# RViMLab/MICCAI2021_Cataract_semantic_segmentation

Hardware: AMD Instinct MI355X
Metric: train frames/sec @540x960 OCRNet-HRNetw48 (higher is better)
Workload: dtype f32 (convolutions with K >= 2048 and >= 192 output columns, and the 3x3 trunk convolutions of the HRNet widths: forward / backward-data of those with > 192 output columns: operands scaled by a per-tensor power of two and split into 2 fp16 planes (22 significant bits), 3 fp16 MFMA products; forward /

## Files before the change

miccai2021_cataract_semantic_segmentation_amd/csrc/pconv1.hip:

```cpp
#include "common.h"

namespace {

typedef _Float16 half8 __attribute__((ext_vector_type(8)));
typedef unsigned short u16;

__host__ __device__ inline int p1_exponent(unsigned amax_bits) {
  const int ex = (int)((amax_bits >> 23) & 0xFF);
  if (ex == 0 || ex == 255) return 0;
  const int e = 14 - (ex - 127);
  return e < -100 ? -100 : (e > 100 ? 100 : e);
}

__host__ __device__ constexpr int p1_bn(int N) { return N >= 256 ? 256 : (N + 31) / 32 * 32; }
__host__ __device__ constexpr int p1_ntn(int N) { return (N + p1_bn(N) - 1) / p1_bn(N); }
__host__ __device__ constexpr int p1_groups(int K) { return ((K + 31) / 32 + 1) / 2 * 2; }

struct P1Entry { long long w_off, img_off; int O, I, kh, kw, transposed, ky0, kys, nky, kx0, kxs, nkx, pad; };

__global__ __launch_bounds__(256) void p1_amax_batch_kernel(const float* __restrict__ flat, const P1Entry* __restrict__ ent, unsigned* __restrict__ recs) {
  const P1Entry e = ent[blockIdx.y];
  const float* w = flat + e.w_off;
  const long long n = (long long)e.O * e.I * e.kh * e.kw;
  unsigned m = 0;
  for (long long i = blockIdx.x * (long long)blockDim.x + threadIdx.x; i < n; i += (long long)gridDim.x * blockDim.x)
    m = max(m, __float_as_uint(w[i]) & 0x7FFFFFFFu);
  cs_amax_commit1(m, recs + 2 * blockIdx.y);
}

__global__ __launch_bounds__(256) void p1_prep_batch_kernel(const float* __restrict__ flat, const P1Entry* __restrict__ ent,
                                                            unsigned char* __restrict__ img_base, unsigned* __restrict__ recs) {
  const P1Entry e = ent[blockIdx.y];
  const int ex = p1_exponent(recs[2 * blockIdx.y]);
  if (blockIdx.x == 0 && threadIdx.x == 0) ((int*)recs)[2 * blockIdx.y + 1] = ex;
  const float* w = flat + e.w_off;
  const int N = e.transposed ? e.I : e.O, Ck = e.transposed ? e.O : e.I, K = e.nky * e.nkx * Ck;
  const int BN = p1_bn(N), ntn = p1_ntn(N), G = p1_groups(K);
  half8* img = (half8*)(img_base + e.img_off);
  const long long pieces = (long long)G * ntn * 2 * BN * 2;
  for (long long i = blockIdx.x * (long long)blockDim.x + threadIdx.x; i < pieces; i += (long long)gridDim.x * blockDim.x) {
    const int c = (int)(i & 1);
    long long r = i >> 1;
    const int nn = (int)(r % BN); r /= BN;
    const int kt = (int)(r & 1); r >>= 1;
    const int nt = (int)(r % ntn);
    const int g = (int)(r / ntn);
    const int n = nt * BN + nn, k0 = 32 * g + 16 * kt + 8 * c;
    half8 h, l;
#pragma unroll
    for (int j = 0; j < 8; ++j) {
      const int k = k0 + j;
      float v = 0.f;
      if (n < N && k < K) {
        const int t = k / Ck, c = k - t * Ck;
        const int ta = t / e.nkx, tb = t - ta * e.nkx;
        const int ky = e.ky0 + ta * e.kys, kx = e.kx0 + tb * e.kxs;
        const int o = e.transposed ? c : n, ci = e.transposed ? n : c;
        v = w[(((long long)o * e.kh + ky) * e.kw + kx) * e.I + ci];
      }
      const float xs = __builtin_ldexpf(v, ex);
      const _Float16 hh = (_Float16)xs;
      h[j] = hh;
      l[j] = (_Float16)(xs - (float)hh);
    }
    const int pc = c ^ ((nn >> 3) & 1);
    const long long row0 = (((long long)(g * ntn + nt) * 2 + kt) * 2) * BN;
    img[(row0 + nn) * 2 + pc] = h;
    img[(row0 + BN + nn) * 2 + pc] = l;
  }
}

struct P1Geo {
  int Wg, HWg;
  int si, y0, x0;
  int ya, xa, nb;
  int Hi, Wi, C;
  unsigned mC, mnb;
  int so, oy, ox, Ho, Wo;
  int linear_out;
};

struct P1Args {
  const float* x; int ldx;
  const unsigned* xrec;
  const unsigned char* wimg;
  const int* wrec;
  float* y; int ldy;
  const float* bias;
  int M, N, K;
  int tilesM, ntn;
  int accumulate;
  float* bn_part;
  unsigned long long x_bytes, img_bytes;
  unsigned long long y_bytes;
  P1Geo geo;
};

template <int NS>
__device__ __forceinline__ void p1_full_tile_bn_partials(float* lds, int tile_cols, int l31, bool writer_lane, int wave_m, const f32x16 (&acc)[NS],
                                                         float* part, int C, int gcol0) {
  constexpr int WM = 8;
  float mean[NS];
#pragma unroll
  for (int j = 0; j < NS; ++j) {
    float a = 0.f;
#pragma unroll
    for (int i = 0; i < 16; ++i) a += acc[j][i];
    a += __shfl_xor(a, 32, 64);
    if (writer_lane) lds[wave_m * tile_cols + 32 * j + l31] = a;
    __builtin_amdgcn_sched_barrier(0);
  }
  __syncthreads();
  const float inv = 1.f / 256.f;
#pragma unroll
  for (int j = 0; j < NS; ++j) {
    float t = 0.f;
#pragma unroll
    for (int w = 0; w < WM; ++w) t += lds[w * tile_cols + 32 * j + l31];
    mean[j] = t * inv;
  }
  __syncthreads();
#pragma unroll
  for (int j = 0; j < NS; ++j) {
    float a = 0.f, b = 0.f;
#pragma unroll
    for (int i = 0; i < 16; ++i) {
      const float d = acc[j][i] - mean[j];
      a += d;
      b += d * d;
    }
    a += __shfl_xor(a, 32, 64);
    b += __shfl_xor(b, 32, 64);
    if (writer_lane) {
      lds[wave_m * tile_cols + 32 * j + l31] = a;
      lds[(WM + wave_m) * tile_cols + 32 * j + l31] = b;
    }
    __builtin_amdgcn_sched_barrier(0);
  }
  __syncthreads();
  if (writer_lane && wave_m == 0) {
#pragma unroll
    for (int j = 0; j < NS; ++j) {
      const int gc = gcol0 + 32 * j + l31;
      if (gc < C) {
        float a = 0.f, b = 0.f;
#pragma unroll
        for (int w = 0; w < WM; ++w) {
          a += lds[w * tile_cols + 32 * j + l31];
          b += lds[(WM + w) * tile_cols + 32 * j + l31];
        }
        part[gc] = mean[j];
        part[C + gc] = a;
        part[2 * C + gc] = b;
      }
    }
  }
}

constexpr int p1_waitcnt(int vm) { return (vm & 15) | (7 << 4) | (15 << 8) | ((vm >> 4) << 14); }

template <int NT, bool GEO, bool FULL>
__device__ __forceinline__ void p1_body(const P1Args& p) {
  constexpr int BN = 32 * NT;
  constexpr int GB = 4 * BN * 32;
  constexpr int PIECES = GB / 16;
  constexpr int PB = (PIECES + 511) / 512;
  constexpr int NBUF = 3;
  constexpr int EPI = 2 * 8 * BN * 4;
  constexpr int SMEM = (NBUF * GB > EPI ? NBUF * GB : EPI) + 1024;
  __shared__ __attribute__((aligned(16))) char smem[SMEM];

  const int tid = threadIdx.x;
  const int lane = tid & 63;
  const int wave = __builtin_amdgcn_readfirstlane(tid >> 6);
  const int l31 = lane & 31, hh = lane >> 5;

  int tile_m = blockIdx.x, tile_n = 0;
  if (p.ntn > 1) {
    const int per = 8 * p.ntn, grp = blockIdx.x / per, r = blockIdx.x - grp * per;
    tile_n = r >> 3;
    tile_m = grp * 8 + (r & 7);
  }
  if (tile_m >= p.tilesM) return;
  const int m0 = tile_m * 256, n0 = tile_n * BN;

  const int ex = p1_exponent(cs_amax_read(p.xrec));
  const int G = p1_groups(p.K);

  f32x16 acc[NT];
#pragma unroll
  for (int u = 0; u < NT; ++u)
#pragma unroll
    for (int r = 0; r < 16; ++r) acc[u][r] = 0.f;

  const __amdgpu_buffer_rsrc_t rsA = __builtin_amdgcn_make_buffer_rsrc((void*)p.x, (short)0, (int)(unsigned)p.x_bytes, 0x00020000);
  const __amdgpu_buffer_rsrc_t rsB = __builtin_amdgcn_make_buffer_rsrc((void*)p.wimg, (short)0, (int)(unsigned)p.img_bytes, 0x00020000);
  constexpr unsigned OOB = 0xFFFFFFF0u;
  const int row = m0 + wave * 32 + l31;
  const unsigned klim = row < p.M ? (unsigned)p.K : 0u;
  unsigned a_row = 0;
  int ybase = 0, xbase = 0;
  if (GEO) {
    const int rr = row < p.M ? row : 0;
    const int gb = rr / p.geo.HWg, rem = rr - gb * p.geo.HWg;
    const int gi = rem / p.geo.Wg, gj = rem - gi * p.geo.Wg;
    ybase = gi * p.geo.si + p.geo.y0;
    xbase = gj * p.geo.si + p.geo.x0;
    a_row = (unsigned)(gb * p.geo.Hi * p.geo.Wi);
  } else {
    a_row = (unsigned)row * (unsigned)p.ldx * 4u + (unsigned)hh * 32u;
  }
  auto a_off = [&](int g, int kt, int c) -> unsigned {
    const unsigned k8 = (unsigned)(32 * g + 16 * kt + 8 * hh);
    if (GEO) {
      const unsigned tap = __umulhi(k8, p.geo.mC), cc = k8 - tap * (unsigned)p.geo.C;
      const unsigned ta = p.geo.nb == 1 ? tap : __umulhi(tap, p.geo.mnb), tb = tap - ta * (unsigned)p.geo.nb;
      const int yi = ybase + (int)ta * p.geo.ya, xi = xbase + (int)tb * p.geo.xa;
      const bool ok = (int)(k8 + 4u * c < klim) & (int)((unsigned)yi < (unsigned)p.geo.Hi) & (int)((unsigned)xi < (unsigned)p.geo.Wi);
      const unsigned m = (unsigned)-(int)ok;
      const unsigned off = ((a_row + (unsigned)(yi * p.geo.Wi + xi)) * (unsigned)p.ldx + cc) * 4u + 16u * c;
      return (off & m) | (OOB & ~m);
    }
    const unsigned m = (unsigned)-(int)(k8 + 4u * c < klim);
    return ((a_row + (unsigned)(32 * g + 16 * kt) * 4u + 16u * c) & m) | (OOB & ~m);
  };
  const unsigned b_lane = (unsigned)(wave * 64 + lane) * 16u;
  auto issueB = [&](int g, int buf) {
    const unsigned src0 = (unsigned)((g * p.ntn + tile_n)) * (unsigned)GB;
#pragma unroll
    for (int i = 0; i < PB; ++i) {
      const bool live = i * 512 + wave * 64 < PIECES;
      const unsigned voff = live ? src0 + (unsigned)i * 8192u + b_lane : OOB;
      char* dst = live ? smem + buf * GB + (i * 512 + wave * 64) * 16 : smem + SMEM - 1024;
      __builtin_amdgcn_raw_ptr_buffer_load_lds(rsB, (__attribute__((address_space(3))) void*)dst, 16, voff, 0, 0, 0);
    }
  };

  f32x4 ra[2][4];
  auto loadA = [&](int g, int par) {
#pragma unroll
    for (int q = 0; q < 4; ++q) ra[par][q] = __builtin_bit_cast(f32x4, __builtin_amdgcn_raw_buffer_load_b128(rsA, a_off(g, q >> 1, q & 1), 0, 0));
  };
  half8 Ah[2], Al[2];
  auto splitA = [&](int par) {
#pragma unroll
    for (int kt = 0; kt < 2; ++kt) {
      const f32x4 v0 = ra[par][kt * 2], v1 = ra[par][kt * 2 + 1];
#pragma unroll
      for (int j = 0; j < 8; ++j) {
        const float xs = __builtin_ldexpf(j < 4 ? v0[j & 3] : v1[j & 3], ex);
        const _Float16 h = (_Float16)xs;
        Ah[kt][j] = h;
        Al[kt][j] = (_Float16)(xs - (float)h);
      }
    }
  };
  const int boff = l31 * 32 + ((hh ^ ((l31 >> 3) & 1)) << 4);
  constexpr int NP = (NT + 1) / 2;
  auto compute = [&](int buf) {
    const char* bb = smem + buf * GB + boff;
    half8 bh[2][2], bl[2][2];
    auto rd = [&](int q, int st) {
      const int kt = q / NP, u = 2 * (q - kt * NP);
      bh[st][0] = *(const half8*)(bb + ((kt * 2 + 0) * BN + 32 * u) * 32);
      bl[st][0] = *(const half8*)(bb + ((kt * 2 + 1) * BN + 32 * u) * 32);
      if (u + 1 < NT) {
        bh[st][1] = *(const half8*)(bb + ((kt * 2 + 0) * BN + 32 * (u + 1)) * 32);
        bl[st][1] = *(const half8*)(bb + ((kt * 2 + 1) * BN + 32 * (u + 1)) * 32);
      }
    };
    rd(0, 0);
#pragma unroll
    for (int q = 0; q < 2 * NP; ++q) {
      const int st = q & 1, kt = q / NP, u = 2 * (q - kt * NP);
      if (q + 1 < 2 * NP) rd(q + 1, st ^ 1);
      if (u + 1 < NT) {
        acc[u] = __builtin_amdgcn_mfma_f32_32x32x16_f16(Al[kt], bh[st][0], acc[u], 0, 0, 0);
        acc[u + 1] = __builtin_amdgcn_mfma_f32_32x32x16_f16(Al[kt], bh[st][1], acc[u + 1], 0, 0, 0);
        acc[u] = __builtin_amdgcn_mfma_f32_32x32x16_f16(Ah[kt], bh[st][0], acc[u], 0, 0, 0);
        acc[u + 1] = __builtin_amdgcn_mfma_f32_32x32x16_f16(Ah[kt], bh[st][1], acc[u + 1], 0, 0, 0);
        acc[u] = __builtin_amdgcn_mfma_f32_32x32x16_f16(Ah[kt], bl[st][0], acc[u], 0, 0, 0);
        acc[u + 1] = __builtin_amdgcn_mfma_f32_32x32x16_f16(Ah[kt], bl[st][1], acc[u + 1], 0, 0, 0);
      } else {
        acc[u] = __builtin_amdgcn_mfma_f32_32x32x16_f16(Al[kt], bh[st][0], acc[u], 0, 0, 0);
        acc[u] = __builtin_amdgcn_mfma_f32_32x32x16_f16(Ah[kt], bh[st][0], acc[u], 0, 0, 0);
        acc[u] = __builtin_amdgcn_mfma_f32_32x32x16_f16(Ah[kt], bl[st][0], acc[u], 0, 0, 0);
      }
      __builtin_amdgcn_sched_barrier(0);
    }
  };

  loadA(0, 0);
  issueB(0, 0);
  loadA(1, 1);
  issueB(1, 1);
  for (int g = 0; g < G; g += 2) {
#pragma unroll
    for (int par = 0; par < 2; ++par) {
      const int gg = g + par;
      splitA(par);
      loadA(gg + 2, par);
      __builtin_amdgcn_sched_barrier(0);
      __builtin_amdgcn_s_waitcnt(p1_waitcnt(8 + PB));
      __builtin_amdgcn_s_barrier();
      asm volatile("" ::: "memory");
      issueB(gg + 2, (gg + 2) % NBUF);
      compute(gg % NBUF);
    }
  }
  __builtin_amdgcn_s_waitcnt(p1_waitcnt(0));
  __syncthreads();

  if constexpr (FULL) {
    const int ew_u = __builtin_amdgcn_readfirstlane(p.wrec[1]), ex_u = __builtin_amdgcn_readfirstlane(ex);
    const int es = -(ex_u + ew_u);
    if (es >= -120 && es <= 120) {
#pragma unroll
      for (int u = 0; u < NT; ++u)
#pragma unroll
        for (int r = 0; r < 16; ++r) acc[u][r] = __builtin_ldexpf(acc[u][r], es);
    } else {
#pragma unroll
      for (int u = 0; u < NT; ++u)
#pragma unroll
        for (int r = 0; r < 16; ++r) acc[u][r] = __builtin_ldexpf(__builtin_ldexpf(acc[u][r], -ex_u), -ew_u);
    }
    if (p.bias != nullptr) {
#pragma unroll
      for (int u = 0; u < NT; ++u) {
        const int col = n0 + 32 * u + l31;
        const float b = col < p.N ? p.bias[col] : 0.f;
#pragma unroll
        for (int r = 0; r < 16; ++r) acc[u][r] += b;
      }
    }
    if (p.bn_part != nullptr)
      p1_full_tile_bn_partials<NT>((float*)smem, BN, l31, hh == 0, wave, acc, p.bn_part + (long long)tile_m * 3 * p.N, p.N, n0);
    constexpr unsigned OOBS = 0xFFFFFFF0u;
    const bool accum = p.accumulate != 0;
    if (GEO && !p.geo.linear_out) {
      const __amdgpu_buffer_rsrc_t rsY = __builtin_amdgcn_make_buffer_rsrc((void*)p.y, (short)0, (int)(unsigned)p.y_bytes, 0x00020000);
      unsigned cb[NT];
#pragma unroll
      for (int u = 0; u < NT; ++u) cb[u] = n0 + 32 * u + l31 < p.N ? (unsigned)(n0 + 32 * u + l31) * 4u : OOBS;
#pragma unroll
      for (int r = 0; r < 16; ++r) {
        const int rw = m0 + wave * 32 + 4 * hh + (r & 3) + 8 * (r >> 2);
        const int gb = rw / p.geo.HWg, rem = rw - gb * p.geo.HWg;
        const int gi = rem / p.geo.Wg, gj = rem - gi * p.geo.Wg;
        const unsigned ro = rw < p.M ? (unsigned)((gb * p.geo.Ho + gi * p.geo.so + p.geo.oy) * p.geo.Wo + gj * p.geo.so + p.geo.ox) * (unsigned)p.ldy * 4u : OOBS;
        float v[NT];
#pragma unroll
        for (int u = 0; u < NT; ++u) v[u] = acc[u][r];
        if (accum) {
          float o[NT];
#pragma unroll
          for (int u = 0; u < NT; ++u) o[u] = __uint_as_float(__builtin_amdgcn_raw_buffer_load_b32(rsY, (cb[u] == OOBS || ro == OOBS) ? OOBS : ro + cb[u], 0, 0));
#pragma unroll
          for (int u = 0; u < NT; ++u) v[u] += o[u];
        }
#pragma unroll
        for (int u = 0; u < NT; ++u) __builtin_amdgcn_raw_buffer_store_b32(__float_as_uint(v[u]), rsY, (cb[u] == OOBS || ro == OOBS) ? OOBS : ro + cb[u], 0, 0);
        __builtin_amdgcn_sched_barrier(0);
      }
      return;
    }
    const unsigned rows_here = (unsigned)(p.M - m0 < 256 ? p.M - m0 : 256);
    const __amdgpu_buffer_rsrc_t rsY = __builtin_amdgcn_make_buffer_rsrc((void*)(p.y + (long long)m0 * p.ldy + n0), (short)0,
                                                                        (int)(rows_here * (unsigned)p.ldy * 4u - (unsigned)n0 * 4u), 0x00020000);
    const int ld4 = p.ldy * 4;
    const int voff = (wave * 32 + 4 * hh) * ld4 + l31 * 4;
    int vo[NT];
#pragma unroll
    for (int u = 0; u < NT; ++u) vo[u] = n0 + 32 * u + l31 < p.N ? voff + 128 * u : (int)OOBS;
#pragma unroll
    for (int r = 0; r < 16; ++r) {
      const int soff = ((r & 3) + 8 * (r >> 2)) * ld4;
      float v[NT];
#pragma unroll
      for (int u = 0; u < NT; ++u) v[u] = acc[u][r];
      if (accum) {
        float o[NT];
#pragma unroll
        for (int u = 0; u < NT; ++u) o[u] = __uint_as_float(__builtin_amdgcn_raw_buffer_load_b32(rsY, vo[u], soff, 0));
#pragma unroll
        for (int u = 0; u < NT; ++u) v[u] += o[u];
      }
#pragma unroll
      for (int u = 0; u < NT; ++u) __builtin_amdgcn_raw_buffer_store_b32(__float_as_uint(v[u]), rsY, vo[u], soff, 0);
      __builtin_amdgcn_sched_barrier(0);
    }
    return;
  }

  {
    const int ea = -ex, ew = -p.wrec[1];
#pragma unroll
    for (int u = 0; u < NT; ++u)
#pragma unroll
      for (int r = 0; r < 16; ++r) acc[u][r] = __builtin_ldexpf(__builtin_ldexpf(acc[u][r], ea), ew);
  }
  float bv[NT];
#pragma unroll
  for (int u = 0; u < NT; ++u) {
    const int col = n0 + 32 * u + l31;
    bv[u] = (p.bias != nullptr && col < p.N) ? p.bias[col] : 0.f;
  }
  const int rbase = m0 + wave * 32 + 4 * hh;
  if (p.bn_part != nullptr) {
    int colv[NT];
#pragma unroll
    for (int u = 0; u < NT; ++u) colv[u] = 32 * u + l31;
    cs_tile_bn_partials<NT, 16, 8, false>(
        (float*)smem, BN, colv, hh == 0, wave, min(256, p.M - m0),
        [&](int j, int i) { return acc[j][i] + bv[j]; },
        [&](int i) { return rbase + (i & 3) + 8 * (i >> 2) < p.M; }, p.bn_part + (long long)tile_m * 3 * p.N, p.N, n0);
  }
  long long orow[16];
#pragma unroll
  for (int r = 0; r < 16; ++r) {
    const int rw = rbase + (r & 3) + 8 * (r >> 2);
    if (GEO && !p.geo.linear_out) {
      const int rr = rw < p.M ? rw : 0;
      const int gb = rr / p.geo.HWg, rem = rr - gb * p.geo.HWg;
      const int gi = rem / p.geo.Wg, gj = rem - gi * p.geo.Wg;
      orow[r] = ((long long)(gb * p.geo.Ho + gi * p.geo.so + p.geo.oy) * p.geo.Wo + gj * p.geo.so + p.geo.ox) * p.ldy;
    } else {
      orow[r] = (long long)rw * p.ldy;
    }
  }
#pragma unroll
  for (int u = 0; u < NT; ++u) {
    const int col = n0 + 32 * u + l31;
    float add[16];
#pragma unroll
    for (int r = 0; r < 16; ++r) {
      const int rw = rbase + (r & 3) + 8 * (r >> 2);
      add[r] = (p.accumulate && rw < p.M && col < p.N) ? p.y[orow[r] + col] : 0.f;
    }
#pragma unroll
    for (int r = 0; r < 16; ++r) {
      const int rw = rbase + (r & 3) + 8 * (r >> 2);
      if (rw < p.M && col < p.N) p.y[orow[r] + col] = (acc[u][r] + bv[u]) + add[r];
    }
  }
}

template <int NT, bool GEO, bool FULL>
__global__ __launch_bounds__(512) void p1_kernel(const P1Args p) {
  p1_body<NT, GEO, FULL>(p);
}
struct P1Multi { P1Args a[4]; };
template <int NT, bool FULL>
__global__ __launch_bounds__(512) void p1_multi_kernel(const P1Multi q) {
  p1_body<NT, true, FULL>(q.a[blockIdx.y]);
}

template <int NT>
void p1_launch_multi(const P1Multi& q, int n, hipStream_t st) {
  int blocks = 0;
  bool full = true;
  for (int i = 0; i < n; ++i) {
    const P1Args& a = q.a[i];
    const int b = a.ntn > 1 ? (a.tilesM + 7) / 8 * 8 * a.ntn : a.tilesM;
    blocks = b > blocks ? b : blocks;
    const bool gathered = !a.geo.linear_out;
    full = full && (gathered ? (a.y_bytes > 0 && a.y_bytes < 0xFFFFFFF0ull) : (a.M % 256 == 0 || a.bn_part == nullptr));
  }
  if (full) hipLaunchKernelGGL((p1_multi_kernel<NT, true>), dim3(blocks, n), dim3(512), 0, st, q);
  else hipLaunchKernelGGL((p1_multi_kernel<NT, false>), dim3(blocks, n), dim3(512), 0, st, q);
}
void p1_dispatch_multi(const P1Multi& q, int n, hipStream_t st) {
  switch (p1_bn(q.a[0].N) / 32) {
    case 1: p1_launch_multi<1>(q, n, st); break;
    case 2: p1_launch_multi<2>(q, n, st); break;
    case 3: p1_launch_multi<3>(q, n, st); break;
    case 4: p1_launch_multi<4>(q, n, st); break;
    case 5: p1_launch_multi<5>(q, n, st); break;
    case 6: p1_launch_multi<6>(q, n, st); break;
    case 7: p1_launch_multi<7>(q, n, st); break;
    default: p1_launch_multi<8>(q, n, st); break;
  }
}

template <int NT>
void p1_launch(const P1Args& a, bool geo, hipStream_t st) {
  const int per = 8 * a.ntn;
  const int blocks = a.ntn > 1 ? (a.tilesM + 7) / 8 * per : a.tilesM;
  const bool gathered = geo && !a.geo.linear_out;
  const bool full = gathered ? (a.y_bytes > 0 && a.y_bytes < 0xFFFFFFF0ull) : (a.M % 256 == 0 || a.bn_part == nullptr);
  if (geo) {
    if (full) hipLaunchKernelGGL((p1_kernel<NT, true, true>), dim3(blocks), dim3(512), 0, st, a);
    else hipLaunchKernelGGL((p1_kernel<NT, true, false>), dim3(blocks), dim3(512), 0, st, a);
  } else {
    if (full) hipLaunchKernelGGL((p1_kernel<NT, false, true>), dim3(blocks), dim3(512), 0, st, a);
    else hipLaunchKernelGGL((p1_kernel<NT, false, false>), dim3(blocks), dim3(512), 0, st, a);
  }
}

void p1_dispatch(const P1Args& a, bool geo, hipStream_t st) {
  switch (p1_bn(a.N) / 32) {
    case 1: p1_launch<1>(a, geo, st); break;
    case 2: p1_launch<2>(a, geo, st); break;
    case 3: p1_launch<3>(a, geo, st); break;
    case 4: p1_launch<4>(a, geo, st); break;
    case 5: p1_launch<5>(a, geo, st); break;
    case 6: p1_launch<6>(a, geo, st); break;
    case 7: p1_launch<7>(a, geo, st); break;
    default: p1_launch<8>(a, geo, st); break;
  }
}

struct P1TArgs {
  const float* dy; int lddy; const unsigned* dyrec;
  const float* x; int ldx; const unsigned* xrec;
  float* slabs;
  long long P;
  int M, N;
  int nbn, Mtot, Ntot;
  int steps_per_block;
  unsigned long long dy_bytes, x_bytes;
  int geo, Cin, kw, stride, pad, dil, Hi, Wi, Ho, Wo;
};

typedef short p1_s16x4 __attribute__((ext_vector_type(4)));
typedef __attribute__((address_space(3))) p1_s16x4 p1_lds_s16x4;

template <int WM, int WN, int TM, int TN, bool GEO>
__global__ __launch_bounds__(512) void p1t_kernel(const P1TArgs p) {
  static_assert(WM * WN == 8, "eight waves");
  constexpr int MP = 32 * TM * WM, NP = 32 * TN * WN;
  constexpr int CH = MP + NP;
  constexpr int RS = (CH * 2 + 63) / 128 * 128 + 64;
  constexpr int PL = 32 * RS;
  __shared__ __attribute__((aligned(16))) char smem[2 * 2 * PL];
  const int tid = threadIdx.x, lane = tid & 63;
  const int wave = __builtin_amdgcn_readfirstlane(tid >> 6);
  const int wm = wave / WN, wn = wave % WN;
  const int edy = p1_exponent(cs_amax_read(p.dyrec)), ex = p1_exponent(cs_amax_read(p.xrec));
  const int bm = blockIdx.y / p.nbn, bn = blockIdx.y - bm * p.nbn;
  const int mo = bm * MP, no = bn * NP;

  f32x16 acc[TM][TN];
#pragma unroll
  for (int i = 0; i < TM; ++i)
#pragma unroll
    for (int j = 0; j < TN; ++j)
#pragma unroll
      for (int r = 0; r < 16; ++r) acc[i][j][r] = 0.f;

  const __amdgpu_buffer_rsrc_t rsD = __builtin_amdgcn_make_buffer_rsrc((void*)p.dy, (short)0, (int)(unsigned)p.dy_bytes, 0x00020000);
  const __amdgpu_buffer_rsrc_t rsX = __builtin_amdgcn_make_buffer_rsrc((void*)p.x, (short)0, (int)(unsigned)p.x_bytes, 0x00020000);
  constexpr unsigned OOB = 0xFFFFFFF0u;
  constexpr int QM = MP / 4, QT = (MP + NP) / 4, QX = QT - QM;
  constexpr int ITD = (32 * QM + 511) / 512, ITX = (32 * QX + 511) / 512, ITEMS = ITD + ITX;
  const long long step0 = (long long)blockIdx.x * p.steps_per_block;
  f32x4 raw[ITEMS];
  auto item = [&](const int i, int& px, int& c4, bool& live) -> bool {
    const bool isx = i >= ITD;
    const int q = (isx ? i - ITD : i) * 512 + tid, Q = isx ? QX : QM;
    px = q / Q;
    c4 = (isx ? QM : 0) + (q - px * Q);
    live = q < 32 * Q;
    return isx;
  };
  int itap[ITEMS];
  const float r_hw = GEO ? 1.f / (float)(p.Ho * p.Wo) : 0.f, r_wo = GEO ? 1.f / (float)p.Wo : 0.f;
  if (GEO) {
#pragma unroll
    for (int i = 0; i < ITEMS; ++i) {
      int px, c4;
      bool live;
      const bool isx = item(i, px, c4, live);
      itap[i] = -1;
      if (live && isx && no + (c4 - QM) * 4 < p.N) {
        const int v = no + (c4 - QM) * 4, tap = v / p.Cin, c = v - tap * p.Cin;
        const int ky = tap / p.kw, kx = tap - ky * p.kw;
        itap[i] = ky | (kx << 8) | (c << 16);
      }
    }
  }
  auto fdiv = [](int n, int d, float rd) -> int {
    int q = (int)((float)n * rd);
    q -= (int)(q * d > n);
    q += (int)((q + 1) * d <= n);
    return q;
  };
  unsigned off0[ITEMS], stepb[ITEMS];
  int pxv[ITEMS];
  if (!GEO) {
#pragma unroll
    for (int i = 0; i < ITEMS; ++i) {
      int px, c4;
      bool live;
      const bool isx = item(i, px, c4, live);
      const bool ok = live && (isx ? (no + (c4 - QM) * 4 < p.N) : (mo + c4 * 4 < p.M));
      const long long pix0 = step0 * 32 + px;
      off0[i] = !ok ? OOB : (isx ? (unsigned)((pix0 * p.ldx + no + (c4 - QM) * 4) * 4) : (unsigned)((pix0 * p.lddy + mo + c4 * 4) * 4));
      stepb[i] = (unsigned)(32 * (isx ? p.ldx : p.lddy) * 4);
      pxv[i] = ok ? px : (1 << 30);
    }
  }
  auto load_plain = [&](int srel) {
    const long long left = p.P - (step0 + srel) * 32;
    const int lim = left > 32 ? 32 : (int)left;
#pragma unroll
    for (int i = 0; i < ITEMS; ++i) {
      const unsigned off = pxv[i] < lim ? off0[i] + (unsigned)srel * stepb[i] : OOB;
      raw[i] = i >= ITD ? __builtin_bit_cast(f32x4, __builtin_amdgcn_raw_buffer_load_b128(rsX, off, 0, 0))
                        : __builtin_bit_cast(f32x4, __builtin_amdgcn_raw_buffer_load_b128(rsD, off, 0, 0));
// ... 460 lines not shown
```

Measured before the change: 83.41.

## Interleave A-operand split and loads with MFMA chain in split-fp16 conv kernel

Restructures the main loop of the split-fp16 pointwise conv kernel so the fp32-to-hi/lo fp16 split of A, the address computation and the global A loads are cut into small pieces and placed between individual MFMA instructions. The A ring grows from 2 to 4 half-group slots, with a deeper prefetch distance and adjusted waitcnt thresholds. The aim is to hide the VALU split work and load issue latency behind the matrix pipeline instead of running them serially before each compute phase. It raises register pressure and relies on hand-tuned waitcnt counts and sched_barrier placement, which could lower occupancy or expose ordering bugs.

```diff
diff --git a/miccai2021_cataract_semantic_segmentation_amd/csrc/pconv1.hip b/miccai2021_cataract_semantic_segmentation_amd/csrc/pconv1.hip
--- a/miccai2021_cataract_semantic_segmentation_amd/csrc/pconv1.hip
+++ b/miccai2021_cataract_semantic_segmentation_amd/csrc/pconv1.hip
@@ -210,19 +210,24 @@
   } else {
     a_row = (unsigned)row * (unsigned)p.ldx * 4u + (unsigned)hh * 32u;
   }
-  auto a_off = [&](int g, int kt, int c) -> unsigned {
-    const unsigned k8 = (unsigned)(32 * g + 16 * kt + 8 * hh);
+  auto a_off2 = [&](int t, unsigned (&off)[2]) {
+    const unsigned k8 = (unsigned)(16 * t + 8 * hh);
+    unsigned base;
+    bool in = true;
     if (GEO) {
       const unsigned tap = __umulhi(k8, p.geo.mC), cc = k8 - tap * (unsigned)p.geo.C;
       const unsigned ta = p.geo.nb == 1 ? tap : __umulhi(tap, p.geo.mnb), tb = tap - ta * (unsigned)p.geo.nb;
       const int yi = ybase + (int)ta * p.geo.ya, xi = xbase + (int)tb * p.geo.xa;
-      const bool ok = (int)(k8 + 4u * c < klim) & (int)((unsigned)yi < (unsigned)p.geo.Hi) & (int)((unsigned)xi < (unsigned)p.geo.Wi);
-      const unsigned m = (unsigned)-(int)ok;
-      const unsigned off = ((a_row + (unsigned)(yi * p.geo.Wi + xi)) * (unsigned)p.ldx + cc) * 4u + 16u * c;
-      return (off & m) | (OOB & ~m);
-    }
-    const unsigned m = (unsigned)-(int)(k8 + 4u * c < klim);
-    return ((a_row + (unsigned)(32 * g + 16 * kt) * 4u + 16u * c) & m) | (OOB & ~m);
+      in = (int)((unsigned)yi < (unsigned)p.geo.Hi) & (int)((unsigned)xi < (unsigned)p.geo.Wi);
+      base = ((a_row + (unsigned)(yi * p.geo.Wi + xi)) * (unsigned)p.ldx + cc) * 4u;
+    } else {
+      base = a_row + (unsigned)(16 * t) * 4u;
+    }
+#pragma unroll
+    for (int c = 0; c < 2; ++c) {
+      const unsigned m = (unsigned)-(int)((int)(k8 + 4u * c < klim) & (int)in);
+      off[c] = ((base + 16u * c) & m) | (OOB & ~m);
+    }
   };
   const unsigned b_lane = (unsigned)(wave * 64 + lane) * 16u;
   auto issueB = [&](int g, int buf) {
@@ -236,76 +241,103 @@
     }
   };
 
-  f32x4 ra[2][4];
-  auto loadA = [&](int g, int par) {
-#pragma unroll
-    for (int q = 0; q < 4; ++q) ra[par][q] = __builtin_bit_cast(f32x4, __builtin_amdgcn_raw_buffer_load_b128(rsA, a_off(g, q >> 1, q & 1), 0, 0));
+  f32x4 ra[4][2];
+  unsigned ao[2];
+  auto loadA = [&](int t, int slot) {
+    a_off2(t, ao);
+#pragma unroll
+    for (int c = 0; c < 2; ++c) ra[slot][c] = __builtin_bit_cast(f32x4, __builtin_amdgcn_raw_buffer_load_b128(rsA, ao[c], 0, 0));
   };
   half8 Ah[2], Al[2];
-  auto splitA = [&](int par) {
-#pragma unroll
-    for (int kt = 0; kt < 2; ++kt) {
-      const f32x4 v0 = ra[par][kt * 2], v1 = ra[par][kt * 2 + 1];
-#pragma unroll
-      for (int j = 0; j < 8; ++j) {
-        const float xs = __builtin_ldexpf(j < 4 ? v0[j & 3] : v1[j & 3], ex);
-        const _Float16 h = (_Float16)xs;
-        Ah[kt][j] = h;
-        Al[kt][j] = (_Float16)(xs - (float)h);
-      }
+  auto split2 = [&](int slot, int fs, int i) {
+#pragma unroll
+    for (int j = 2 * i; j < 2 * i + 2; ++j) {
+      const float xs = __builtin_ldexpf(ra[slot][j >> 2][j & 3], ex);
+      const _Float16 h = (_Float16)xs;
+      Ah[fs][j] = h;
+      Al[fs][j] = (_Float16)(xs - (float)h);
     }
   };
   const int boff = l31 * 32 + ((hh ^ ((l31 >> 3) & 1)) << 4);
   constexpr int NP = (NT + 1) / 2;
-  auto compute = [&](int buf) {
-    const char* bb = smem + buf * GB + boff;
-    half8 bh[2][2], bl[2][2];
-    auto rd = [&](int q, int st) {
-      const int kt = q / NP, u = 2 * (q - kt * NP);
-      bh[st][0] = *(const half8*)(bb + ((kt * 2 + 0) * BN + 32 * u) * 32);
-      bl[st][0] = *(const half8*)(bb + ((kt * 2 + 1) * BN + 32 * u) * 32);
+  constexpr int NM = 3 * NT;
+  constexpr int NW = 6;
+  half8 bh[2][2], bl[2][2];
+  auto rdB = [&](const char* bb, int kt, int q) {
+    const int st = (kt * NP + q) & 1, u = 2 * q;
+    bh[st][0] = *(const half8*)(bb + ((kt * 2 + 0) * BN + 32 * u) * 32);
+    bl[st][0] = *(const half8*)(bb + ((kt * 2 + 1) * BN + 32 * u) * 32);
+    if (u + 1 < NT) {
+      bh[st][1] = *(const half8*)(bb + ((kt * 2 + 0) * BN + 32 * (u + 1)) * 32);
+      bl[st][1] = *(const half8*)(bb + ((kt * 2 + 1) * BN + 32 * (u + 1)) * 32);
+    }
+  };
+  auto p1_half = [&](const char* bb, int t, int kt, int slot) {
+    int m = 0;
+    auto work = [&]() {
+#pragma unroll
+      for (int w = 0; w < NW; ++w)
+        if (w * NM / NW == m) {
+          __builtin_amdgcn_sched_barrier(0);
+          if (w == 0 && kt == 1) __builtin_amdgcn_s_waitcnt(p1_waitcnt(2 * PB + 6));
+          if (w < 4) split2(slot, kt ^ 1, w);
+          else if (w == 4) a_off2(t + 5, ao);
+          else {
+#pragma unroll
+            for (int c = 0; c < 2; ++c) ra[slot][c] = __builtin_bit_cast(f32x4, __builtin_amdgcn_raw_buffer_load_b128(rsA, ao[c], 0, 0));
+          }
+          __builtin_amdgcn_sched_barrier(0);
+        }
+      ++m;
+    };
+    auto mm = [&](f32x16& c, const half8& a, const half8& b) {
+      c = __builtin_amdgcn_mfma_f32_32x32x16_f16(a, b, c, 0, 0, 0);
+      work();
+    };
+#pragma unroll
+    for (int q = 0; q < NP; ++q) {
+      const int st = (kt * NP + q) & 1, u = 2 * q;
+      if (q + 1 < NP) rdB(bb, kt, q + 1);
+      else if (kt == 0) rdB(bb, 1, 0);
+      __builtin_amdgcn_sched_barrier(0);
       if (u + 1 < NT) {
-        bh[st][1] = *(const half8*)(bb + ((kt * 2 + 0) * BN + 32 * (u + 1)) * 32);
-        bl[st][1] = *(const half8*)(bb + ((kt * 2 + 1) * BN + 32 * (u + 1)) * 32);
-      }
-    };
-    rd(0, 0);
-#pragma unroll
-    for (int q = 0; q < 2 * NP; ++q) {
-      const int st = q & 1, kt = q / NP, u = 2 * (q - kt * NP);
-      if (q + 1 < 2 * NP) rd(q + 1, st ^ 1);
-      if (u + 1 < NT) {
-        acc[u] = __builtin_amdgcn_mfma_f32_32x32x16_f16(Al[kt], bh[st][0], acc[u], 0, 0, 0);
-        acc[u + 1] = __builtin_amdgcn_mfma_f32_32x32x16_f16(Al[kt], bh[st][1], acc[u + 1], 0, 0, 0);
-        acc[u] = __builtin_amdgcn_mfma_f32_32x32x16_f16(Ah[kt], bh[st][0], acc[u], 0, 0, 0);
-        acc[u + 1] = __builtin_amdgcn_mfma_f32_32x32x16_f16(Ah[kt], bh[st][1], acc[u + 1], 0, 0, 0);
-        acc[u] = __builtin_amdgcn_mfma_f32_32x32x16_f16(Ah[kt], bl[st][0], acc[u], 0, 0, 0);
-        acc[u + 1] = __builtin_amdgcn_mfma_f32_32x32x16_f16(Ah[kt], bl[st][1], acc[u + 1], 0, 0, 0);
+        mm(acc[u], Al[kt], bh[st][0]);
+        mm(acc[u + 1], Al[kt], bh[st][1]);
+        mm(acc[u], Ah[kt], bh[st][0]);
+        mm(acc[u + 1], Ah[kt], bh[st][1]);
+        mm(acc[u], Ah[kt], bl[st][0]);
+        mm(acc[u + 1], Ah[kt], bl[st][1]);
       } else {
-        acc[u] = __builtin_amdgcn_mfma_f32_32x32x16_f16(Al[kt], bh[st][0], acc[u], 0, 0, 0);
-        acc[u] = __builtin_amdgcn_mfma_f32_32x32x16_f16(Ah[kt], bh[st][0], acc[u], 0, 0, 0);
-        acc[u] = __builtin_amdgcn_mfma_f32_32x32x16_f16(Ah[kt], bl[st][0], acc[u], 0, 0, 0);
-      }
-      __builtin_amdgcn_sched_barrier(0);
+        mm(acc[u], Al[kt], bh[st][0]);
+        mm(acc[u], Ah[kt], bh[st][0]);
+        mm(acc[u], Ah[kt], bl[st][0]);
+      }
     }
   };
 
   loadA(0, 0);
   issueB(0, 0);
   loadA(1, 1);
+  loadA(2, 2);
   issueB(1, 1);
+  loadA(3, 3);
+#pragma unroll
+  for (int i = 0; i < 4; ++i) split2(0, 0, i);
+  loadA(4, 0);
+  __builtin_amdgcn_sched_barrier(0);
   for (int g = 0; g < G; g += 2) {
 #pragma unroll
     for (int par = 0; par < 2; ++par) {
       const int gg = g + par;
-      splitA(par);
-      loadA(gg + 2, par);
       __builtin_amdgcn_sched_barrier(0);
-      __builtin_amdgcn_s_waitcnt(p1_waitcnt(8 + PB));
+      __builtin_amdgcn_s_waitcnt(p1_waitcnt(PB + 6));
       __builtin_amdgcn_s_barrier();
       asm volatile("" ::: "memory");
       issueB(gg + 2, (gg + 2) % NBUF);
-      compute(gg % NBUF);
+      const char* bb = smem + (gg % NBUF) * GB + boff;
+      rdB(bb, 0, 0);
+      p1_half(bb, 2 * gg, 0, 2 * par + 1);
+      p1_half(bb, 2 * gg + 1, 1, (2 * par + 2) & 3);
     }
   }
   __builtin_amdgcn_s_waitcnt(p1_waitcnt(0));
```

Result: no change. 83.36 (-0.1%).
